# loop-Z/omniisaacgymenvs_loop

Hardware: AMD Instinct MI355X
Metric: env-steps/sec USV_CaptureXY at 1/2/4/8 MI355X; wall-clock to reward=30 (higher is better)
Workload: dtype fp32; 1 GPU; USV_Virtual_CaptureXY num_envs=131072/GPU PPO-MLP fp32 (BASELINE configs[4] per GPU: 2^20 envs over 8 GPUs); num_envs_per_gpu=131072, horizon_length=16, minibatch_size=8192, mini_epochs=8, parallelism=dp1, exchange=none (one rank), seed=0, full=False

## Files before the change

omniisaacgymenvs_loop_amd/csrc/ppo.hip:

```cpp
#include <cstdlib>
#include <cstring>
#include <type_traits>

#include "usv_device.h"

USV_PROBE_DEFINE(ppo)
USV_PROBE_DEFINE(pol)
USV_PROBE_DEFINE(red)

namespace {

constexpr int NIN = PPO_NIN, NH = PPO_NH, NA = PPO_NA;
constexpr int RB = 32;
constexpr int TB = 256;
constexpr int XS = 35;
constexpr int HS = 129;
constexpr int NPART = PPO_NPARAM + 8;
constexpr int NPART_PAD = (NPART + 3) & ~3;
constexpr int P_LOSS = PPO_NPARAM;
constexpr float kLog2Pi = 1.8378770664093453f;

typedef float f32x16 __attribute__((ext_vector_type(16)));
typedef unsigned int u32x4_t __attribute__((ext_vector_type(4)));

// ... 797 lines not shown
#pragma unroll
      for (int u = 0; u < 8; ++u) xv[u] = obs[(size_t)min(r0 + u * nl, bnd - 1) * NIN + col];
#pragma unroll
      for (int u = 0; u < 8; ++u)
        if (r0 + u * nl < bnd) {
          const double x = xv[u];
          s += x; s2 += x * x;
        }
    }
    acc[0][col][lane_r] = s;
    acc[1][col][lane_r] = s2;
  }
  __syncthreads();
  if (tid < NIN) {
    double t = 0, t2 = 0;
    for (int l = 0; l < nl; ++l) { t += acc[0][tid][l]; t2 += acc[1][tid][l]; }
    double *o = part + ((size_t)mb * OM_CH + ch) * 2 * NIN;
    o[tid] = t;
    o[NIN + tid] = t2;
  }
}

constexpr int RS_TB = 256, RS_U = 8;
__global__ __launch_bounds__(RS_TB) void k_obs_rms_seq(ppo_cfg_t c, const double *__restrict__ part, int nmb,
                                                       double *obs_rms, double *seq) {
  const double rows = (double)c.minibatch;
  for (int q = threadIdx.x; q < nmb * NIN; q += RS_TB) {
    const int mb = q / NIN, k = q % NIN;
    double sa = 0, sb = 0;
#pragma unroll
    for (int ch = 0; ch < OM_CH; ++ch) {
      const double *o = part + ((size_t)mb * OM_CH + ch) * 2 * NIN;
      sa += o[k];
      sb += o[NIN + k];
    }
    const double bmean = sa / rows;
    seq[(size_t)mb * 2 * NIN + k] = bmean;
    seq[(size_t)mb * 2 * NIN + NIN + k] = (sb - rows * bmean * bmean) / (rows - 1.0);
  }
  __syncthreads();
  const int k = threadIdx.x;
  if (k < NIN) {
    double mean = obs_rms[k], var = obs_rms[NIN + k], count = obs_rms[2 * NIN];
    for (int mb0 = 0; mb0 < nmb; mb0 += RS_U) {
      double bm[RS_U], bv[RS_U];
#pragma unroll
      for (int u = 0; u < RS_U; ++u) {
        const int mb = min(mb0 + u, nmb - 1);
        bm[u] = seq[(size_t)mb * 2 * NIN + k];
        bv[u] = seq[(size_t)mb * 2 * NIN + NIN + k];
      }
#pragma unroll
      for (int u = 0; u < RS_U; ++u) {
        if (mb0 + u >= nmb) break;
        const double tot = count + rows;
        const double delta = bm[u] - mean;
        const double M2 = var * count + bv[u] * rows + delta * delta * count * rows / tot;
        mean = mean + delta * rows / tot;
        var = M2 / tot;
        count = tot;
        seq[(size_t)(mb0 + u) * 2 * NIN + k] = mean;
        seq[(size_t)(mb0 + u) * 2 * NIN + NIN + k] = var;
      }
    }
    obs_rms[k] = mean;
    obs_rms[NIN + k] = var;
    if (k == 0) obs_rms[2 * NIN] = count;
  }
}

constexpr int GTB = 512;

#ifndef USV_RD_P
#define USV_RD_P 128
#endif
typedef float f32x4v __attribute__((ext_vector_type(4)));
constexpr int RD_TB = 512, RD_P = USV_RD_P;
constexpr int RD_L = RD_P / 4;
constexpr int RD_G = (RD_TB / RD_L);
constexpr int RD_KB = 16;
constexpr int RED_BLOCKS = (PPO_NPARAM + 5 + RD_P - 1) / RD_P;
static_assert(RD_P % 4 == 0 && 64 % RD_L == 0 && RD_P <= RD_TB, "reduce geometry");
static_assert(RED_BLOCKS <= 256, "chunk squares: one per thread of waves 0-3");

struct AdamBanks {
  const float *P0, *m0, *v0;
  float *P1, *m1, *v1;
};
struct AdamK {
  float step_size, bc2s;
};
__device__ __forceinline__ AdamK adam_consts(const ppo_cfg_t &c, float lr, float step) {
  const double bc1 = 1.0 - pow((double)c.adam_b1, (double)step);
  const double bc2 = 1.0 - pow((double)c.adam_b2, (double)step);
  return {(float)((double)lr / bc1), (float)sqrt(bc2)};
}
__device__ __forceinline__ void adam_one(const ppo_cfg_t &c, const AdamK &k, float g, float p_old, float m_old,
                                         float v_old, float &pn, float &mn, float &vn) {
  if (c.weight_decay != 0.f) g = g + c.weight_decay * p_old;
  mn = m_old + (1.0f - c.adam_b1) * (g - m_old);
  vn = v_old * c.adam_b2 + (1.0f - c.adam_b2) * g * g;
  const float denom = sqrtf(vn) / k.bc2s + c.adam_eps;
  pn = p_old - k.step_size * (mn / denom);
}
__device__ __forceinline__ float clip_coef(const ppo_cfg_t &c, float total_norm) {
  float coef = 1.0f;
  if (c.truncate_grads) {
    coef = c.grad_norm / (total_norm + 1e-6f);
    coef = fminf(coef, 1.0f);
  }
  return coef;
}
__device__ __forceinline__ AdamK adam_consts_tagged(const ppo_cfg_t &c, float lr, float step, float t_ss,
                                                    float t_bc, float t_step, float t_lr) {
  if (t_step == step && t_lr == lr) return {t_ss, t_bc};
  return adam_consts(c, lr, step);
}
struct OptNext {
  float nl, kl_keep, step;
  AdamK nk;
};
template <class OptIn>
__device__ __forceinline__ OptNext opt_next(const ppo_cfg_t &c, const OptIn &opt_in, float kl) {
  const float lr = opt_in[0];
  float nl = lr, kl_keep = opt_in[2];
  if (c.lr_adaptive) {
    if (kl > 2.0f * c.kl_threshold) nl = fmaxf(lr / 1.5f, c.lr_min);
    if (kl < 0.5f * c.kl_threshold) nl = fminf(lr * 1.5f, c.lr_max);
    kl_keep = kl;
  }
  const float step = opt_in[1] + 1.0f;
  return {nl, kl_keep, step, adam_consts(c, nl, step + 1.0f)};
}
__device__ __forceinline__ void opt_store(const ppo_cfg_t &c, const OptNext &x, float *opt_out, float total_norm,
                                          float kl, float *kl_out) {
  if (c.lr_adaptive && kl_out) *kl_out = kl;
  opt_out[0] = x.nl;
  opt_out[1] = x.step;
  opt_out[2] = x.kl_keep;
  opt_out[3] = total_norm;
  opt_out[4] = x.nk.step_size;
  opt_out[5] = x.nk.bc2s;
  opt_out[6] = x.step + 1.0f;
  opt_out[7] = x.nl;
}

struct ChainIn {
  const float *P_prev, *m_prev, *v_prev;
  float *P_cur, *m_cur, *v_cur;
  const float *grad;
  const float *opt_prev;
  float *opt_cur;
  float *kl_out;
  uint32_t *dp_clock;
  int fold_skip;
  float gscale;
};

constexpr int XG = XS;
constexpr int GX = ((RB * XG + GTB - 1) / GTB) * GTB;
struct GradSmem {
  float w2[NH * HS];
  float w1[NH * XG];
  float x[GX];
  float h1[RB * HS];
  float h2[RB * HS];
  float xch[4][16][64];
  float out[RB * 4];
  float g[RB * 4];
  float hg[4][4][NH];
  float b1[NH];
  float tail[TAIL + 1];
  float nrm[4];
  int fold[2];
};

constexpr int S_W2 = 0, S_W1 = NH * NH, S_SIG = S_W1 + NH * 32, S_B1 = S_SIG + 2, S_TAIL = S_B1 + NH,
              S_W1C = S_TAIL + TAIL, S_END = S_W1C + NH;
static_assert(S_END == PPO_NPARAM && S_W1 % 4 == 0 && NIN == 33, "partial slot layout");
__device__ __forceinline__ int tail_slot(int param) { return S_TAIL + param - PPO_OFF_B2; }
__device__ __forceinline__ int acc_slot(int base, int tile, int a, int lane) { return base + ((tile * 4 + a) * 64 + lane) * 4; }
__device__ __forceinline__ int param_of_slot(int s) {
  if (s < S_W1) {
    const int tile = s >> 10, a = (s >> 8) & 3, lane = (s >> 2) & 63, q = 4 * a + (s & 3);
    const int n = 32 * (tile >> 2) + crow(q, lane >> 5), k = 32 * (tile & 3) + (lane & 31);
    return PPO_OFF_W2 + n * NH + k;
  }
  if (s < S_SIG) {
    const int t = s - S_W1, tile = t >> 10, a = (t >> 8) & 3, lane = (t >> 2) & 63, q = 4 * a + (t & 3);
    const int n = 32 * tile + crow(q, lane >> 5), k = lane & 31;
    return PPO_OFF_W1 + n * NIN + k;
  }
  if (s < S_B1) return PPO_OFF_SIGMA + (s - S_SIG);
  if (s < S_TAIL) return PPO_OFF_B1 + (s - S_B1);
  if (s < S_W1C) return PPO_OFF_B2 + (s - S_TAIL);
  if (s < S_END) return PPO_OFF_W1 + (s - S_W1C) * NIN + (NIN - 1);
  return -1;
}

struct RowIn {
  float act0, act1, nlp, val, ret, adv, mu0, mu1, sg0, sg1;
};

#ifndef USV_PART_AUX
#define USV_PART_AUX 2
#endif
template <int kAux, bool kCM>
struct PartOutT {
  __amdgpu_buffer_rsrc_t r;
  uint32_t cs;
  __device__ __forceinline__ uint32_t off(int idx) const {
    if constexpr (kCM) return (uint32_t)(idx / RD_P) * cs + (uint32_t)(idx % RD_P) * 4u;
    else return (uint32_t)idx * 4u;
  }
  __device__ __forceinline__ void operator()(int idx, float v) const {
    __builtin_amdgcn_raw_buffer_store_b32(__builtin_bit_cast(uint32_t, v), r, off(idx), 0, kAux);
  }
  __device__ __forceinline__ void x4(int idx, float a, float b, float c, float d) const {
    const u32x4_t v = {__builtin_bit_cast(uint32_t, a), __builtin_bit_cast(uint32_t, b), __builtin_bit_cast(uint32_t, c),
                       __builtin_bit_cast(uint32_t, d)};
    __builtin_amdgcn_raw_buffer_store_b128(v, r, off(idx), 0, kAux);
  }
};
constexpr int AUX_SC1 = 16;

constexpr int FOLD_G = 8;
static_assert(RD_G >= FOLD_G, "k_reduce_partials(fold = 1) reads one group row per row group");
constexpr int FOLD_MAX_M = 32;
constexpr int FOLD_CTL_STRIDE = 64;
constexpr uint64_t FOLD_WAIT_TICKS = 10000;
__host__ __device__ constexpr size_t part_body_floats(int nblk) {
  return (size_t)nblk * RED_BLOCKS * RD_P > (size_t)(nblk + FOLD_G) * NPART_PAD ? (size_t)nblk * RED_BLOCKS * RD_P
                                                                                 : (size_t)(nblk + FOLD_G) * NPART_PAD;
}
__device__ __forceinline__ uint32_t *fold_ctl(float *partials, int nblk) {
  return reinterpret_cast<uint32_t *>(partials + part_body_floats(nblk));
}
__device__ __forceinline__ const uint32_t *fold_ctl(const float *partials, int nblk) {
  return reinterpret_cast<const uint32_t *>(partials + part_body_floats(nblk));
}
__device__ __forceinline__ f32x4v ld4_sc1(__amdgpu_buffer_rsrc_t r, uint32_t byte_off) {
  return __builtin_bit_cast(f32x4v, __builtin_amdgcn_raw_buffer_load_b128(r, byte_off, 0, AUX_SC1));
}

__device__ __forceinline__ void redo_step(const ppo_cfg_t &c, const ChainIn &ch, const float (&op)[8], float coef,
                                          float scale, GradSmem &s, float &ls0, float &ls1) {
  const AdamK ak = adam_consts_tagged(c, op[0], op[1] + 1.0f, op[4], op[5], op[6], op[7]);
  for (int q = threadIdx.x; q < PPO_NPARAM; q += GTB) {
    float pn, mn, vn;
    adam_one(c, ak, ch.grad[q] * scale * coef, ch.P_prev[q], ch.m_prev[q], ch.v_prev[q], pn, mn, vn);
    if ((q / GTB) % gridDim.x == blockIdx.x) {
      ch.P_cur[q] = pn; ch.m_cur[q] = mn; ch.v_cur[q] = vn;
    }
    if (q >= PPO_OFF_B2) {
      s.tail[q - PPO_OFF_B2] = pn;
    } else if (q >= PPO_OFF_W2) {
      const int e = q - PPO_OFF_W2;
      s.w2[(e / NH) * HS + e % NH] = pn;
    } else if (q >= PPO_OFF_B1) {
      s.b1[q - PPO_OFF_B1] = pn;
    } else if (q >= PPO_OFF_W1) {
      const int e = q - PPO_OFF_W1;
      s.w1[(e / NIN) * XG + e % NIN] = pn;
    }
  }
  float pn, mn, vn;
  adam_one(c, ak, ch.grad[PPO_OFF_SIGMA] * scale * coef, ch.P_prev[PPO_OFF_SIGMA], ch.m_prev[PPO_OFF_SIGMA],
           ch.v_prev[PPO_OFF_SIGMA], pn, mn, vn);
  ls0 = pn;
  adam_one(c, ak, ch.grad[PPO_OFF_SIGMA + 1] * scale * coef, ch.P_prev[PPO_OFF_SIGMA + 1],
           ch.m_prev[PPO_OFF_SIGMA + 1], ch.v_prev[PPO_OFF_SIGMA + 1], pn, mn, vn);
  ls1 = pn;
}

constexpr int APN_TB = 256;
__device__ __forceinline__ float apply_norm_part(const float *__restrict__ grad_in, float grad_scale, int tid) {
  constexpr int N4 = PPO_NPARAM / 4, U = (N4 + APN_TB - 1) / APN_TB;
  const float4 *g4 = reinterpret_cast<const float4 *>(grad_in);
  float4 gv[U];
#pragma unroll
  for (int u = 0; u < U; ++u) gv[u] = g4[min(tid + u * APN_TB, N4 - 1)];
  float ss = 0.f;
#pragma unroll
  for (int u = 0; u < U; ++u) {
    if (tid + u * APN_TB >= N4) continue;
    const float x = gv[u].x * grad_scale, y = gv[u].y * grad_scale;
    const float z = gv[u].z * grad_scale, w = gv[u].w * grad_scale;
    ss = fmaf(x, x, ss); ss = fmaf(y, y, ss); ss = fmaf(z, z, ss); ss = fmaf(w, w, ss);
  }
  for (int r = 4 * N4 + tid; r < PPO_NPARAM; r += APN_TB) {
    const float g = grad_in[r] * grad_scale;
    ss = fmaf(g, g, ss);
  }
  return ss;
}

template <bool kBf, bool kChain, bool kFold, bool kColl = false>
__device__ __forceinline__ void mb_grad8w(const ppo_cfg_t &c, const ChainIn &ch, const float *__restrict__ P,
                                          const double *__restrict__ obs_rms, int row0,
                                          const float *__restrict__ e_obs, const float *__restrict__ e_act,
                                          const float *__restrict__ e_nlp, const float *__restrict__ e_val,
                                          const float *__restrict__ e_ret, const float *__restrict__ e_adv,
                                          float *e_mu, float *e_sigma, float *partials, GradSmem &s) {
  const int tid = threadIdx.x, lane = tid & 63, w = tid >> 6;
  const int i = lane & 31, h = lane >> 5;
  const int kh = w >> 2, cb = w & 3, n0 = 32 * cb;
  const int rb0 = row0 + blockIdx.x * RB;
  const float invB = 1.0f / (float)c.minibatch;
  USV_PHASE(ppo, 0);
  if (ch.dp_clock && blockIdx.x == 0 && tid == 0) *ch.dp_clock += 1u;
  constexpr int NW1G = (NH * XG + GTB - 1) / GTB, NTLG = (TAIL + GTB - 1) / GTB, NW2F = NH * NH / GTB;
  static_assert(NH * NH % GTB == 0, "staging trip counts");
  float w2f[NW2F];
  float w1r[NW1G], tlr[NTLG];
  float ov = 0.f;
  if constexpr (kChain) ov = lane < 8 ? ch.opt_prev[lane] : ch.grad[PPO_NPARAM];
  {
#pragma unroll
    for (int u = 0; u < NW1G; ++u) {
      const int q = min(tid + u * GTB, NH * XG - 1), j = q / XG, k = q % XG;
      w1r[u] = P[PPO_OFF_W1 + j * NIN + min(k, NIN - 1)];
    }
#pragma unroll
    for (int u = 0; u < NTLG; ++u) tlr[u] = P[PPO_OFF_B2 + min(tid + u * GTB, TAIL - 1)];
  }
  const float b1r = P[PPO_OFF_B1 + (tid & (NH - 1))];
  const float lsv = P[PPO_OFF_SIGMA + (lane & 1)];
  float lsig0 = 0.f, lsig1 = 0.f;
  float csq = 0.f;
  if constexpr (kChain) csq = ch.grad[PPO_NPARAM + 8 + min(tid, RED_BLOCKS - 1)];
  RowIn ri;
  {
    const size_t row = (size_t)rb0 + (lane & (RB - 1));
    ri.act0 = e_act[row * 2]; ri.act1 = e_act[row * 2 + 1];
    ri.nlp = e_nlp[row]; ri.adv = e_adv[row];
    ri.val = e_val[row]; ri.ret = e_ret[row];
    ri.mu0 = e_mu[row * 2]; ri.mu1 = e_mu[row * 2 + 1];
    ri.sg0 = e_sigma[row * 2]; ri.sg1 = e_sigma[row * 2 + 1];
  }
  constexpr int NU = (RB * XG + GTB - 1) / GTB;
  float xo[NU];
  double mu[NU], var[NU];
#pragma unroll
  for (int u = 0; u < NU; ++u) {
    const int q = min(tid + u * GTB, RB * XG - 1), r = q / XG, kc = min(q % XG, NIN - 1);
    xo[u] = e_obs[(size_t)(rb0 + r) * NIN + kc];
    mu[u] = obs_rms[kc];
    var[u] = obs_rms[NIN + kc];
  }
#pragma unroll
  for (int u = 0; u < NW2F; ++u) w2f[u] = P[PPO_OFF_W2 + tid + u * GTB];
  __builtin_amdgcn_sched_barrier(0);
#pragma unroll
  for (int u = 0; u < NW1G; ++u)
    if ((tid + u * GTB) % XG >= NIN) w1r[u] = 0.f;
  if (kChain && tid >= RED_BLOCKS) csq = 0.f;
  {
    const bool norm = c.normalize_input != 0;
#pragma unroll
    for (int u = 0; u < NU; ++u) {
      const int q = tid + u * GTB;
      const int k = q % XG;
      const float xn = rms_norm(xo[u], mu[u], var[u], c.rms_eps);
      const float xv = (k < NIN && q < RB * XG) ? (norm ? xn : xo[u]) : 0.f;
      s.x[q] = xv;
    }
  }
#pragma unroll
  for (int u = 0; u < NW1G; ++u)
    if (tid + u * GTB < NH * XG) s.w1[tid + u * GTB] = w1r[u];
#pragma unroll
  for (int u = 0; u < NTLG; ++u)
    if (tid + u * GTB < TAIL) s.tail[tid + u * GTB] = tlr[u];
  if (tid < NH) s.b1[tid] = b1r;
  if (kChain && !kColl && w < 4) {
    const float t = wave_sum(csq);
    if (lane == 0) s.nrm[w] = t;
  }
  __syncthreads();
  if constexpr (kColl) {
    if (w < 4) {
      const float t = wave_sum(apply_norm_part(ch.grad, ch.gscale, tid));
      if (lane == 0) s.nrm[w] = t;
    }
    __syncthreads();
  }
  bool slow = false;
  if constexpr (kChain) {
    const auto lane_of = [&](int q) {
      return __builtin_bit_cast(float, __builtin_amdgcn_readlane(__builtin_bit_cast(int, ov), q));
    };
    const float total_norm = sqrtf(((s.nrm[0] + s.nrm[1]) + s.nrm[2]) + s.nrm[3]);
    const float coef = clip_coef(c, total_norm);
    const float gscale = kColl ? ch.gscale : 1.0f;
    if (blockIdx.x == 0 && tid == 256) {
      float op[8];
#pragma unroll
      for (int q = 0; q < 8; ++q) op[q] = lane_of(q);
      const float kl_prev = kColl ? lane_of(8) * gscale : lane_of(8);
      opt_store(c, opt_next(c, op, kl_prev), ch.opt_cur, total_norm, kl_prev, ch.kl_out);
    }
    if (kColl || coef < 1.0f) {
      slow = true;
      float op[8];
#pragma unroll
      for (int q = 0; q < 8; ++q) op[q] = lane_of(q);
      redo_step(c, ch, op, coef, gscale, s, lsig0, lsig1);
      __syncthreads();
    }
  }
  USV_PHASE(ppo, 1);
  if (kh == 0) {
    f32x16 acc = {};
#pragma unroll
    for (int st = 0; st < 17; ++st) {
      const int k = 2 * st + h;
      acc = mfma32(s.x[i * XG + k], s.w1[(n0 + i) * XG + k], acc);
    }
    const float bj = s.b1[n0 + i];
#pragma unroll
    for (int r = 0; r < 16; ++r) s.h1[crow(r, h) * HS + n0 + i] = fast_tanh(acc[r] + bj);
  }
  USV_PHASE(ppo, 9);
  if (!slow) {
#pragma unroll
    for (int u = 0; u < NW2F; ++u) {
      const int e = tid + u * GTB;
      s.w2[(e >> 7) * HS + (e & (NH - 1))] = w2f[u];
    }
  }
  __syncthreads();
  USV_PHASE(ppo, 10);
  const int ra = (i + 16 * kh) & (RB - 1);
  {
    f32x16 acc = {};
    if constexpr (kBf) {
#pragma unroll
      for (int st = 0; st < NH / 32; ++st) {
        const int k0 = 64 * kh + 16 * st + 8 * h;
        acc = mfma_bf16(ld8(&s.h1[ra * HS + k0]), ld8(&s.w2[(n0 + i) * HS + k0]), acc);
      }
    } else {
#pragma unroll 16
      for (int st = 0; st < NH / 4; ++st) {
        const int k = 64 * kh + 2 * st + h;
        acc = mfma32(s.h1[ra * HS + k], s.w2[(n0 + i) * HS + k], acc);
      }
    }
    USV_PHASE(ppo, 11);
#pragma unroll
    for (int q = 0; q < 8; ++q) s.xch[cb][8 * kh + q][lane] = acc[8 + q];
    __syncthreads();
    const float bj = s.tail[T_B2 + n0 + i];
#pragma unroll
    for (int q = 0; q < 8; ++q)
      s.h2[(crow(q, h) + 16 * kh) * HS + n0 + i] = fast_tanh((acc[q] + s.xch[cb][8 - 8 * kh + q][lane]) + bj);
  }
  __syncthreads();
  USV_PHASE(ppo, 12);
  constexpr bool kCM = !kFold;
  const PartOutT<kFold ? AUX_SC1 : USV_PART_AUX, kCM> part_st{
      kCM ? __builtin_amdgcn_make_buffer_rsrc(partials + (size_t)blockIdx.x * RD_P, 0,
                                              (int)(((size_t)RED_BLOCKS * gridDim.x - blockIdx.x) * RD_P * 4), 0x00020000)
          : __builtin_amdgcn_make_buffer_rsrc(partials + (size_t)blockIdx.x * NPART_PAD, 0, NPART * 4, 0x00020000),
      (uint32_t)gridDim.x * RD_P * 4u};
  {
    const int r = tid / 16, part = tid % 16;
    float a0 = 0.f, a1 = 0.f, av = 0.f;
#pragma unroll
    for (int kk = 0; kk < 8; ++kk) {
      const int k = part + 16 * kk;
      const float hv = s.h2[r * HS + k];
      a0 = fmaf(s.tail[T_WMU + k], hv, a0);
      a1 = fmaf(s.tail[T_WMU + NH + k], hv, a1);
      av = fmaf(s.tail[T_WV + k], hv, av);
    }
#pragma unroll
    for (int m = 1; m < 16; m <<= 1) {
      a0 += __shfl_xor(a0, m, 64);
      a1 += __shfl_xor(a1, m, 64);
      av += __shfl_xor(av, m, 64);
    }
    if (part == 0) {
      s.out[r * 4 + 0] = a0 + s.tail[T_BMU];
      s.out[r * 4 + 1] = a1 + s.tail[T_BMU + 1];
      s.out[r * 4 + 2] = av + s.tail[T_BV];
    }
  }
  __syncthreads();
  USV_PHASE(ppo, 2);
  if (tid < 192) {
    const int r = lane;
    const bool rowok = r < RB;
    const int rr = rowok ? r : 0;
    const size_t row = (size_t)rb0 + rr;
    const float mu0 = s.out[rr * 4], mu1 = s.out[rr * 4 + 1], v = s.out[rr * 4 + 2];
    if (!slow) {
      lsig0 = __builtin_bit_cast(float, __builtin_amdgcn_readlane(__builtin_bit_cast(int, lsv), 0));
      lsig1 = __builtin_bit_cast(float, __builtin_amdgcn_readlane(__builtin_bit_cast(int, lsv), 1));
    }
    const float ls0 = mu0 * 0.f + lsig0, ls1 = mu1 * 0.f + lsig1;
    const float sg0 = expf(ls0), sg1 = expf(ls1);
    const float bh0 = fmaxf(mu0 - 1.1f, 0.f), bl0 = fminf(mu0 + 1.1f, 0.f);
    const float bh1 = fmaxf(mu1 - 1.1f, 0.f), bl1 = fminf(mu1 + 1.1f, 0.f);
    if (w == 0) {
      float la = 0.f, gs0 = 0.f, gs1 = 0.f;
      if (rowok) {
// ... 363 lines not shown
  const int p4 = blockIdx.x * RD_L + col;
  const bool ok = p4 < NPART_PAD / 4;
  const float4 *P4 = reinterpret_cast<const float4 *>(partials);
  const int myslot = blockIdx.x * RD_P + tid;
  const bool mine = kSpec && tid < RD_P && myslot < S_END;
  const int pq = mine ? param_of_slot(myslot) : 0;
  float p_old = 0.f, m_old = 0.f, v_old = 0.f;
  if (mine) {
    p_old = a.P0[pq]; m_old = a.m0[pq]; v_old = a.v0[pq];
  }
  uint32_t key = 0u;
  if (kDP) key = *dp.clock;
  float4 acc = make_float4(0.f, 0.f, 0.f, 0.f);
  float oin[8] = {};
  if (kSpec) {
#pragma unroll
    for (int q = 0; q < 8; ++q) oin[q] = opt_in[q];
  }
  const int p4c = min(p4, NPART_PAD / 4 - 1);
  if (fold) {
    if (grp < FOLD_G) {
      const int M = nblk / FOLD_G;
      const uint32_t *ctl = fold_ctl(partials, nblk) + grp * FOLD_CTL_STRIDE;
      const uint32_t gen = ctl[0] / (uint32_t)M;
      bool folded = true;
      for (int mm = 0; mm < M; ++mm) folded &= ctl[32 + mm] == gen;
      if (folded) {
        acc = P4[(size_t)(nblk + grp) * (NPART_PAD / 4) + p4c];
      } else {
        const int h0 = (M + 1) / 2;
        float4 a0 = make_float4(0.f, 0.f, 0.f, 0.f), a1 = a0;
        for (int mm = 0; mm < M; ++mm) {
          const float4 x = P4[(size_t)(grp + FOLD_G * mm) * (NPART_PAD / 4) + p4c];
          float4 &t = mm < h0 ? a0 : a1;
          t.x += x.x; t.y += x.y; t.z += x.z; t.w += x.w;
        }
        acc = make_float4(a0.x + a1.x, a0.y + a1.y, a0.z + a1.z, a0.w + a1.w);
      }
    }
  } else
  for (int b0 = grp; b0 < nblk; b0 += RD_G * RD_KB) {
    float4 x[RD_KB];
#pragma unroll
    for (int k = 0; k < RD_KB; ++k) {
      const int row = min(b0 + RD_G * k, nblk - 1);
      const float4 *src = P4 + ((size_t)blockIdx.x * nblk + row) * RD_L + col;
      const f32x4v v = __builtin_nontemporal_load(reinterpret_cast<const f32x4v *>(src));
      x[k] = make_float4(v[0], v[1], v[2], v[3]);
    }
#pragma unroll
    for (int k = 0; k < RD_KB; ++k) {
      if (ok && b0 + RD_G * k < nblk) {
        acc.x += x[k].x; acc.y += x[k].y; acc.z += x[k].z; acc.w += x[k].w;
      }
    }
  }
  USV_PHASE(red, 1);
  AdamK ak = {0.f, 1.f};
  if (kSpec)
    ak = adam_consts_tagged(c, oin[0], oin[1] + 1.0f, oin[4], oin[5], oin[6], oin[7]);
  red[grp][col] = acc;
  __syncthreads();
  float s = 0.f;
  const int slot = blockIdx.x * RD_P + tid;
  if (tid < RD_P) {
#pragma unroll
    for (int g = 0; g < RD_G; ++g) s += reinterpret_cast<const float *>(red[g])[tid];
  }
  USV_PHASE(red, 2);
  float sl = s;
  if constexpr (kDP) {
    const float pv = slot < S_END ? s : (slot == PPO_NPARAM + 4 ? s * inv_b : 0.f);
    s = dp_exchange(dp, key, blockIdx.x, slot, pv, dp.timeout_ms) / (float)dp.world;
  }
  float sq = 0.f;
  if (tid < RD_P) {
    if (slot < S_END) {
      grad[param_of_slot(slot)] = s;
      sq = s * s;
      if (mine) {
        float pn, mn, vn;
        adam_one(c, ak, s, p_old, m_old, v_old, pn, mn, vn);
        a.P1[pq] = pn; a.m1[pq] = mn; a.v1[pq] = vn;
      }
    } else if (slot < PPO_NPARAM + 5) {
      const int q = slot - PPO_NPARAM;
      if (q == 4) grad[PPO_NPARAM] = kDP ? s : s * inv_b;
      if (losses) losses[q] = sl * inv_b;
    }
  }
  USV_PHASE(red, 3);
  if (w < (RD_P + 63) / 64) {
    sq = wave_sum(sq);
    if (lane == 0) sqw[w] = sq;
  }
  __syncthreads();
  if (tid == 0) {
    float t = 0.f;
#pragma unroll
    for (int q = 0; q < (RD_P + 63) / 64; ++q) t += sqw[q];
    grad[PPO_NPARAM + 8 + blockIdx.x] = t;
  }
  USV_PHASE(red, 4);
}

constexpr int AP_TB = 256;
template <bool kNormFromPartials, bool kFinish>
__global__ __launch_bounds__(AP_TB) void k_apply(ppo_cfg_t c, AdamBanks a, const float *__restrict__ grad_in,
                                                 const float *__restrict__ opt_in, float *__restrict__ opt_out,
                                                 float grad_scale, float *kl_out) {
  __shared__ float red[AP_TB / 64];
  const int tid = threadIdx.x;
  const int q = blockIdx.x * AP_TB + tid;
  const int qc = min(q, PPO_NPARAM - 1);
  const float g_raw = grad_in[qc], p_old = a.P0[qc], m_old = a.m0[qc], v_old = a.v0[qc];
  const float s0 = grad_in[PPO_NPARAM + 8 + min(tid, RED_BLOCKS - 1)];
  const float lr = opt_in[0];
  const float step = opt_in[1] + 1.0f;
  const float kl = grad_in[PPO_NPARAM] * grad_scale;
  __builtin_amdgcn_sched_barrier(0);
  const AdamK ak = adam_consts_tagged(c, lr, step, opt_in[4], opt_in[5], opt_in[6], opt_in[7]);
  OptNext nx = {};
  if (blockIdx.x == 0 && tid == 0) nx = opt_next(c, opt_in, kl);
  __asm__ volatile("" : : "v"(ak.step_size), "v"(ak.bc2s), "v"(nx.nl), "v"(nx.nk.step_size), "v"(nx.nk.bc2s));
  float ss = 0.f;
  if (kNormFromPartials) {
    ss = tid < RED_BLOCKS ? s0 : 0.f;
  } else {
    constexpr int N4 = PPO_NPARAM / 4, U = (N4 + AP_TB - 1) / AP_TB;
    const float4 *g4 = reinterpret_cast<const float4 *>(grad_in);
    float4 gv[U];
#pragma unroll
    for (int u = 0; u < U; ++u) gv[u] = g4[min(tid + u * AP_TB, N4 - 1)];
#pragma unroll
    for (int u = 0; u < U; ++u) {
      if (tid + u * AP_TB >= N4) continue;
      const float x = gv[u].x * grad_scale, y = gv[u].y * grad_scale;
      const float z = gv[u].z * grad_scale, w = gv[u].w * grad_scale;
      ss = fmaf(x, x, ss); ss = fmaf(y, y, ss); ss = fmaf(z, z, ss); ss = fmaf(w, w, ss);
    }
    for (int r = 4 * N4 + tid; r < PPO_NPARAM; r += AP_TB) {
      const float g = grad_in[r] * grad_scale;
      ss = fmaf(g, g, ss);
    }
  }
  ss = wave_sum(ss);
  if ((tid & 63) == 0) red[tid >> 6] = ss;
  __syncthreads();
  const float total_norm = sqrtf(((red[0] + red[1]) + red[2]) + red[3]);
  const float coef = clip_coef(c, total_norm);
  if (q < PPO_NPARAM && (!kFinish || coef < 1.0f)) {
    float pn, mn, vn;
    adam_one(c, ak, g_raw * grad_scale * coef, p_old, m_old, v_old, pn, mn, vn);
    a.P1[q] = pn;
    a.m1[q] = mn;
    a.v1[q] = vn;
  }
  if (blockIdx.x == 0 && tid == 0) opt_store(c, nx, opt_out, total_norm, kl, kl_out);
}

}

extern "C" {

int ppo_policy_step(const ppo_cfg_t *cfg, const float *params, const double *obs_rms, const double *val_rms,
                    const float *obs, int t, float *exp_obs, float *exp_act, float *exp_nlp, float *exp_val,
// ... 48 lines not shown
                const float *last_obs, const int64_t *last_dones, const uint8_t *exp_done, float *exp_val,
                const float *exp_rew, float *exp_ret, float *exp_adv, double *work, void *stream) {
  if (!cfg || !params || !work || cfg->n_envs <= 0) return 1;
  hipStream_t s = (hipStream_t)stream;
  float *last_val = reinterpret_cast<float *>(work + 8 + 8 * 4096);
  if (ppo_value(cfg, params, obs_rms, val_rms, last_obs, last_val, stream)) return 2;
  const int nblk = (cfg->n_envs + TB - 1) / TB;
  if (nblk > 4096) return 3;
  const char *gv = getenv("USV_GAE_VEC");
  const bool vec16 = !(gv && atoi(gv) == 0) && cfg->horizon == 16 &&
                     ((reinterpret_cast<uintptr_t>(exp_val) | reinterpret_cast<uintptr_t>(exp_rew) |
                       reinterpret_cast<uintptr_t>(exp_ret) | reinterpret_cast<uintptr_t>(exp_adv) |
                       reinterpret_cast<uintptr_t>(exp_done)) & 15u) == 0;
  hipLaunchKernelGGL(vec16 ? k_gae<16> : k_gae<0>, dim3(nblk), dim3(TB), 0, s, *cfg, last_val, last_dones, exp_done,
                     exp_val, exp_rew, exp_ret, exp_adv, work);
  USV_CHECK_LAUNCH();
  hipLaunchKernelGGL(k_prepare_finalize, dim3(1), dim3(FIN_TB), 0, s, *cfg, val_rms, work, nblk);
  USV_CHECK_LAUNCH();
  const size_t B = (size_t)cfg->n_envs * cfg->horizon;
  hipLaunchKernelGGL(k_prepare_apply, dim3((unsigned)((B + 255) / 256)), dim3(256), 0, s, *cfg, work, exp_val,
                     exp_ret, exp_adv);
  USV_CHECK_LAUNCH();
  return 0;
}

static int fold_env() {
  const char *e = getenv("USV_PPO_FOLD");
  return e ? atoi(e) : 0;
}
static bool fold_on(int nblk) {
  return fold_env() != 0 && nblk % FOLD_G == 0 && nblk / FOLD_G >= 1 && nblk / FOLD_G <= FOLD_MAX_M;
}

int ppo_minibatch_grad(const ppo_cfg_t *cfg, const float *params, double *obs_rms, const double *val_rms,
                       int update_obs_rms, int mb_index, const float *exp_obs, const float *exp_act,
                       const float *exp_nlp, const float *exp_val, const float *exp_ret, const float *exp_adv,
                       float *exp_mu, float *exp_sigma, float *grad, float *losses, float *partials, double *work,
                       void *stream) {
  (void)val_rms;
  if (!cfg || !params || !obs_rms || !grad || !partials || !work) return 1;
  if (cfg->minibatch % RB != 0 || ppo_partials_floats(cfg->minibatch) <= 0) return 2;
  if (reinterpret_cast<uintptr_t>(params) & 15u) return 4;
  hipStream_t s = (hipStream_t)stream;
  const int row0 = mb_index * cfg->minibatch;
  if (update_obs_rms && cfg->normalize_input) {
    const int nb = 64;
    hipLaunchKernelGGL(k_obs_stats, dim3(nb), dim3(TB), 0, s, *cfg, exp_obs, row0, cfg->minibatch, work + 8, obs_rms,
                       reinterpret_cast<unsigned *>(work + 7));
    USV_CHECK_LAUNCH();
  }
  if (reinterpret_cast<uintptr_t>(partials) & 15u) return 3;
  const int nblk = cfg->minibatch / RB;
  const bool fold = fold_on(nblk);
  ChainIn ch{};
  ch.fold_skip = fold_env() == 2;
  hipLaunchKernelGGL((cfg->bf16_gemm ? (fold ? k_mb_grad<true, false, true> : k_mb_grad<true, false, false>)
                                     : (fold ? k_mb_grad<false, false, true> : k_mb_grad<false, false, false>)),
                     dim3(nblk), dim3(GTB), 0, s, *cfg, ch, params, obs_rms, row0, exp_obs, exp_act, exp_nlp,
                     exp_val, exp_ret, exp_adv, exp_mu, exp_sigma, partials);
  USV_CHECK_LAUNCH();
  hipLaunchKernelGGL((k_reduce_partials<false, false>), dim3(RED_BLOCKS), dim3(RD_TB), 0, s, partials, nblk, grad,
                     losses, 1.0f / (float)cfg->minibatch, *cfg, AdamBanks{}, nullptr, ppo_dp_t{}, (int)fold);
  USV_CHECK_LAUNCH();
  return 0;
}

static bool banks_ok(const ppo_adam_banks_t *b) {
  if (!b || !b->opt) return false;
  for (int i = 0; i < 2; ++i) {
    if (!b->params[i] || !b->m[i] || !b->v[i]) return false;
    if (reinterpret_cast<uintptr_t>(b->params[i]) & 15u) return false;
  }
  return true;
}

static int fused_launch(const ppo_cfg_t *cfg, const ppo_adam_banks_t *banks, const ppo_dp_t *dp, int seq,
                        double *obs_rms, int update_obs_rms, int mb_index, const float *exp_obs, const float *exp_act,
                        const float *exp_nlp, const float *exp_val, const float *exp_ret, const float *exp_adv,
                        float *exp_mu, float *exp_sigma, float *grad, float *losses, float *partials, double *work,
                        float *kl_prev_out, void *stream) {
  if (!cfg || !obs_rms || !grad || !partials || !work || seq < 0) return 1;
  if (!banks_ok(banks)) return 4;
  if (cfg->minibatch % RB != 0 || ppo_partials_floats(cfg->minibatch) <= 0) return 2;
  if (reinterpret_cast<uintptr_t>(partials) & 15u) return 3;
  if (dp) {
    if (dp->world < 1 || dp->world > PPO_DP_MAX || dp->rank < 0 || dp->rank >= dp->world || !dp->clock || !dp->err)
      return 5;
    for (int r = 0; r < dp->world; ++r)
      if (!dp->peer[r]) return 5;
  }
  hipStream_t s = (hipStream_t)stream;
  const int cur = seq & 1, prv = cur ^ 1, nblk = cfg->minibatch / RB, row0 = mb_index * cfg->minibatch;
  if (update_obs_rms && cfg->normalize_input) {
    hipLaunchKernelGGL(k_obs_stats, dim3(64), dim3(TB), 0, s, *cfg, exp_obs, row0, cfg->minibatch, work + 8, obs_rms,
                       reinterpret_cast<unsigned *>(work + 7));
    USV_CHECK_LAUNCH();
  }
  const float *P = banks->params[cur];
  const dim3 gg(nblk), gb(GTB);
  uint32_t *clk = dp ? dp->clock : nullptr;
  const bool fold = fold_on(nblk);
  if (seq == 0) {
    ChainIn ch{};
    ch.dp_clock = clk;
    ch.fold_skip = fold_env() == 2;
    hipLaunchKernelGGL((cfg->bf16_gemm ? (fold ? k_mb_grad<true, false, true> : k_mb_grad<true, false, false>)
                                       : (fold ? k_mb_grad<false, false, true> : k_mb_grad<false, false, false>)),
                       gg, gb, 0, s, *cfg, ch, P, obs_rms, row0, exp_obs, exp_act, exp_nlp, exp_val, exp_ret, exp_adv,
                       exp_mu, exp_sigma, partials);
  } else {
    const ChainIn ch{banks->params[prv], banks->m[prv], banks->v[prv], banks->params[cur], banks->m[cur],
                     banks->v[cur], grad, banks->opt + 8 * prv, banks->opt + 8 * cur, kl_prev_out, clk,
                     fold_env() == 2};
    hipLaunchKernelGGL((cfg->bf16_gemm ? (fold ? k_mb_grad<true, true, true> : k_mb_grad<true, true, false>)
                                       : (fold ? k_mb_grad<false, true, true> : k_mb_grad<false, true, false>)),
                       gg, gb, 0, s, *cfg, ch, P, obs_rms, row0, exp_obs, exp_act, exp_nlp, exp_val, exp_ret, exp_adv,
                       exp_mu, exp_sigma, partials);
  }
  USV_CHECK_LAUNCH();
  const AdamBanks a{banks->params[cur], banks->m[cur], banks->v[cur], banks->params[prv], banks->m[prv],
                    banks->v[prv]};
  if (dp)
    hipLaunchKernelGGL((k_reduce_partials<true, true>), dim3(RED_BLOCKS), dim3(RD_TB), 0, s, partials, nblk, grad,
                       losses, 1.0f / (float)cfg->minibatch, *cfg, a, banks->opt + 8 * cur, *dp, (int)fold);
  else
    hipLaunchKernelGGL((k_reduce_partials<true, false>), dim3(RED_BLOCKS), dim3(RD_TB), 0, s, partials, nblk, grad,
                       losses, 1.0f / (float)cfg->minibatch, *cfg, a, banks->opt + 8 * cur, ppo_dp_t{}, (int)fold);
  USV_CHECK_LAUNCH();
  return 0;
}

int ppo_minibatch_fused(const ppo_cfg_t *cfg, const ppo_adam_banks_t *banks, int seq, double *obs_rms,
                        int update_obs_rms, int mb_index, const float *exp_obs, const float *exp_act,
                        const float *exp_nlp, const float *exp_val, const float *exp_ret, const float *exp_adv,
                        float *exp_mu, float *exp_sigma, float *grad, float *losses, float *partials, double *work,
                        float *kl_prev_out, void *stream) {
  return fused_launch(cfg, banks, nullptr, seq, obs_rms, update_obs_rms, mb_index, exp_obs, exp_act, exp_nlp, exp_val,
                      exp_ret, exp_adv, exp_mu, exp_sigma, grad, losses, partials, work, kl_prev_out, stream);
}

int ppo_minibatch_fused_dp(const ppo_cfg_t *cfg, const ppo_adam_banks_t *banks, const ppo_dp_t *dp, int seq,
                           double *obs_rms, int update_obs_rms, int mb_index, const float *exp_obs,
                           const float *exp_act, const float *exp_nlp, const float *exp_val, const float *exp_ret,
                           const float *exp_adv, float *exp_mu, float *exp_sigma, float *grad, float *losses,
                           float *partials, double *work, float *kl_prev_out, void *stream) {
  if (!dp) return 5;
  return fused_launch(cfg, banks, dp, seq, obs_rms, update_obs_rms, mb_index, exp_obs, exp_act, exp_nlp, exp_val,
                      exp_ret, exp_adv, exp_mu, exp_sigma, grad, losses, partials, work, kl_prev_out, stream);
}

int ppo_minibatch_coll(const ppo_cfg_t *cfg, const ppo_adam_banks_t *banks, int seq, float grad_scale,
                       double *obs_rms, int update_obs_rms, int mb_index, const float *exp_obs, const float *exp_act,
                       const float *exp_nlp, const float *exp_val, const float *exp_ret, const float *exp_adv,
                       float *exp_mu, float *exp_sigma, float *grad, float *losses, float *partials, double *work,
                       float *kl_prev_out, void *stream) {
  if (!cfg || !obs_rms || !grad || !partials || !work || seq < 0 || !(grad_scale > 0.f)) return 1;
  if (!banks_ok(banks)) return 4;
  if (cfg->minibatch % RB != 0 || ppo_partials_floats(cfg->minibatch) <= 0) return 2;
  if ((reinterpret_cast<uintptr_t>(partials) | reinterpret_cast<uintptr_t>(grad)) & 15u) return 3;
  hipStream_t s = (hipStream_t)stream;
  const int cur = seq & 1, prv = cur ^ 1, nblk = cfg->minibatch / RB, row0 = mb_index * cfg->minibatch;
  if (update_obs_rms && cfg->normalize_input) {
    hipLaunchKernelGGL(k_obs_stats, dim3(64), dim3(TB), 0, s, *cfg, exp_obs, row0, cfg->minibatch, work + 8, obs_rms,
                       reinterpret_cast<unsigned *>(work + 7));
    USV_CHECK_LAUNCH();
  }
  const float *P = banks->params[cur];
// ... 43 lines not shown
  hipLaunchKernelGGL(k_dp_selftest, dim3(RED_BLOCKS), dim3(RD_TB), 0, (hipStream_t)stream, *dp, (uint32_t)key0,
                     rounds, timeout_ms);
  USV_CHECK_LAUNCH();
  return 0;
}

int ppo_dp_alloc(void **dptr, void *ipc_handle) {
  if (!dptr || !ipc_handle) return 1;
  static_assert(sizeof(hipIpcMemHandle_t) == 64, "ipc handle size");
  const char *mode = getenv("USV_DP_MALLOC");
  const bool plain = mode && strcmp(mode, "plain") == 0;
  if (plain || hipExtMallocWithFlags(dptr, (size_t)DP_BYTES, hipDeviceMallocUncached) != hipSuccess) {
    (void)hipGetLastError();
    if (hipMalloc(dptr, (size_t)DP_BYTES) != hipSuccess) return 2;
  }
  if (hipMemset(*dptr, 0, (size_t)DP_BYTES) != hipSuccess || hipDeviceSynchronize() != hipSuccess) return 3;
  hipIpcMemHandle_t h;
  if (hipIpcGetMemHandle(&h, *dptr) != hipSuccess) return 4;
  memcpy(ipc_handle, &h, sizeof(h));
  return 0;
}

int ppo_dp_open(const void *ipc_handle, void **dptr) {
  if (!dptr || !ipc_handle) return 1;
  hipIpcMemHandle_t h;
  memcpy(&h, ipc_handle, sizeof(h));
  return hipIpcOpenMemHandle(dptr, h, hipIpcMemLazyEnablePeerAccess) == hipSuccess ? 0 : 2;
}

int ppo_dp_close(void *dptr) { return hipIpcCloseMemHandle(dptr) == hipSuccess ? 0 : 1; }
int ppo_dp_free(void *dptr) { return hipFree(dptr) == hipSuccess ? 0 : 1; }

int ppo_minibatch_finish(const ppo_cfg_t *cfg, const ppo_adam_banks_t *banks, int count, const float *grad,
                         float *kl_out, void *stream) {
  if (!cfg || !grad || count <= 0) return 1;
  if (!banks_ok(banks)) return 4;
  const int last = (count - 1) & 1, nxt = last ^ 1;
  const AdamBanks a{banks->params[last], banks->m[last], banks->v[last], banks->params[nxt], banks->m[nxt],
                    banks->v[nxt]};
  hipLaunchKernelGGL((k_apply<true, true>), dim3((PPO_NPARAM + AP_TB - 1) / AP_TB), dim3(AP_TB), 0,
                     (hipStream_t)stream, *cfg, a, grad, banks->opt + 8 * last, banks->opt + 8 * nxt, 1.0f, kl_out);
  USV_CHECK_LAUNCH();
  return 0;
}

int ppo_rms_seq_doubles(const ppo_cfg_t *cfg, int rows) {
  if (!cfg || cfg->minibatch <= 0 || rows < cfg->minibatch) return -1;
  const int nmb = rows / cfg->minibatch;
  return nmb * 2 * NIN + nmb * OM_CH * 2 * NIN;
}

int ppo_obs_rms_epoch(const ppo_cfg_t *cfg, const float *exp_obs, int rows, double *obs_rms, double *rms_seq,
                      void *stream) {
  if (!cfg || !exp_obs || !obs_rms || !rms_seq || cfg->minibatch <= 1 || rows < cfg->minibatch) return 1;
  const int nmb = rows / cfg->minibatch;
  hipStream_t s = (hipStream_t)stream;
  double *part = rms_seq + (size_t)nmb * 2 * NIN;
  hipLaunchKernelGGL(k_obs_moments, dim3(nmb, OM_CH), dim3(TB), 0, s, *cfg, exp_obs, part);
  USV_CHECK_LAUNCH();
  hipLaunchKernelGGL(k_obs_rms_seq, dim3(1), dim3(RS_TB), 0, s, *cfg, part, nmb, obs_rms, rms_seq);
  USV_CHECK_LAUNCH();
  return 0;
}

int ppo_minibatch_apply(const ppo_cfg_t *cfg, float *params, float *grad, float *adam_m, float *adam_v, float *opt,
                        int opt_slot, float grad_scale, float *kl_out, int norm_from_partials, void *stream) {
  if (!cfg || !params || !grad || !adam_m || !adam_v || !opt) return 1;
  if (reinterpret_cast<uintptr_t>(grad) & 15u) return 2;
  if (opt_slot != 0 && opt_slot != 1) return 3;
  const AdamBanks a{params, adam_m, adam_v, params, adam_m, adam_v};
  hipLaunchKernelGGL((norm_from_partials ? k_apply<true, false> : k_apply<false, false>),
                     dim3((PPO_NPARAM + AP_TB - 1) / AP_TB), dim3(AP_TB), 0, (hipStream_t)stream, *cfg, a, grad,
                     opt + 8 * opt_slot, opt + 8 * (1 - opt_slot), grad_scale, kl_out);
  USV_CHECK_LAUNCH();
  return 0;
}

int ppo_partials_floats(int minibatch) {
  static_assert(RED_BLOCKS * RD_P >= NPART_PAD, "chunk-major rows cover a partial row");
  if (minibatch < RB || minibatch % RB != 0) return -1;
  const long long f = (long long)part_body_floats(minibatch / RB) + FOLD_G * FOLD_CTL_STRIDE;
  return f > 0x7fffffffLL ? -1 : (int)f;
}
int ppo_grad_floats(void) { return PPO_NPARAM + 8 + RED_BLOCKS; }
int ppo_meter_floats(int n_envs, int horizon) {
  return horizon * 4 + horizon * ((n_envs + kStoreTB - 1) / kStoreTB) * 4;
}

}
```

Baseline: 35.36 million env-steps/s.

## Stage W2 into LDS via direct global-to-LDS DMA from padded image

The reduce/Adam kernel now also writes updated W2 weights into a padded, LDS-layout image appended to the grad buffer. The chained gradient kernel then copies that image straight into shared memory with global_load_lds_dwordx4, instead of loading W2 into registers and scattering it to LDS later. This is meant to cut register pressure and the VGPR-to-LDS store pass, and to overlap the W2 load with the layer-1 compute. In exchange it adds extra global writes in the reduce kernel, a larger grad buffer, inline asm that touches m0, and explicit vmcnt waits.

```diff
diff --git a/omniisaacgymenvs_loop_amd/csrc/ppo.hip b/omniisaacgymenvs_loop_amd/csrc/ppo.hip
--- a/omniisaacgymenvs_loop_amd/csrc/ppo.hip
+++ b/omniisaacgymenvs_loop_amd/csrc/ppo.hip
@@ -903,6 +903,12 @@
 constexpr int RED_BLOCKS = (PPO_NPARAM + 5 + RD_P - 1) / RD_P;
 static_assert(RD_P % 4 == 0 && 64 % RD_L == 0 && RD_P <= RD_TB, "reduce geometry");
 static_assert(RED_BLOCKS <= 256, "chunk squares: one per thread of waves 0-3");
+constexpr int W2IMG_FLOATS = (NH * HS + 3) & ~3;
+constexpr int W2IMG_OFF = (PPO_NPARAM + 8 + RED_BLOCKS + 3) & ~3;
+constexpr int W2IMG_PIECES = W2IMG_FLOATS / 256;
+constexpr int W2IMG_LAST_LANES = W2IMG_FLOATS % 256 / 4;
+static_assert(W2IMG_FLOATS == NH * HS && W2IMG_PIECES % 8 == 0 && W2IMG_LAST_LANES > 0 && W2IMG_LAST_LANES < 64,
+              "W2 image: the copy covers s.w2 exactly, 8 waves x whole pieces + one partial piece");
 
 struct AdamBanks {
   const float *P0, *m0, *v0;
@@ -981,7 +987,7 @@
 constexpr int XG = XS;
 constexpr int GX = ((RB * XG + GTB - 1) / GTB) * GTB;
 struct GradSmem {
-  float w2[NH * HS];
+  alignas(16) float w2[NH * HS];
   float w1[NH * XG];
   float x[GX];
   float h1[RB * HS];
@@ -1062,6 +1068,15 @@
 }
 __device__ __forceinline__ f32x4v ld4_sc1(__amdgpu_buffer_rsrc_t r, uint32_t byte_off) {
   return __builtin_bit_cast(f32x4v, __builtin_amdgcn_raw_buffer_load_b128(r, byte_off, 0, AUX_SC1));
+}
+
+__device__ __forceinline__ void lds_dma16(const float *src, uint32_t lds_dst) {
+  uint32_t keep;
+  __asm__ volatile("s_mov_b32 %0, m0\n\ts_mov_b32 m0, %2\n\ts_nop 0\n\tglobal_load_lds_dwordx4 %1, off\n\t"
+                   "s_mov_b32 m0, %0"
+                   : "=&s"(keep)
+                   : "v"(src), "s"(lds_dst)
+                   : "memory");
 }
 
 __device__ __forceinline__ void redo_step(const ppo_cfg_t &c, const ChainIn &ch, const float (&op)[8], float coef,
@@ -1132,7 +1147,8 @@
   if (ch.dp_clock && blockIdx.x == 0 && tid == 0) *ch.dp_clock += 1u;
   constexpr int NW1G = (NH * XG + GTB - 1) / GTB, NTLG = (TAIL + GTB - 1) / GTB, NW2F = NH * NH / GTB;
   static_assert(NH * NH % GTB == 0, "staging trip counts");
-  float w2f[NW2F];
+  constexpr bool kImg = kChain && !kColl && !kFold;
+  float w2f[kImg ? 1 : NW2F];
   float w1r[NW1G], tlr[NTLG];
   float ov = 0.f;
   if constexpr (kChain) ov = lane < 8 ? ch.opt_prev[lane] : ch.grad[PPO_NPARAM];
@@ -1146,19 +1162,21 @@
     for (int u = 0; u < NTLG; ++u) tlr[u] = P[PPO_OFF_B2 + min(tid + u * GTB, TAIL - 1)];
   }
   const float b1r = P[PPO_OFF_B1 + (tid & (NH - 1))];
-  const float lsv = P[PPO_OFF_SIGMA + (lane & 1)];
+  float lsv;
+  if constexpr (!kImg) lsv = P[PPO_OFF_SIGMA + (lane & 1)];
   float lsig0 = 0.f, lsig1 = 0.f;
   float csq = 0.f;
   if constexpr (kChain) csq = ch.grad[PPO_NPARAM + 8 + min(tid, RED_BLOCKS - 1)];
   RowIn ri;
-  {
+  const auto load_rows = [&] {
     const size_t row = (size_t)rb0 + (lane & (RB - 1));
     ri.act0 = e_act[row * 2]; ri.act1 = e_act[row * 2 + 1];
     ri.nlp = e_nlp[row]; ri.adv = e_adv[row];
     ri.val = e_val[row]; ri.ret = e_ret[row];
     ri.mu0 = e_mu[row * 2]; ri.mu1 = e_mu[row * 2 + 1];
     ri.sg0 = e_sigma[row * 2]; ri.sg1 = e_sigma[row * 2 + 1];
-  }
+  };
+  if constexpr (!kImg) load_rows();
   constexpr int NU = (RB * XG + GTB - 1) / GTB;
   float xo[NU];
   double mu[NU], var[NU];
@@ -1169,8 +1187,23 @@
     mu[u] = obs_rms[kc];
     var[u] = obs_rms[NIN + kc];
   }
-#pragma unroll
-  for (int u = 0; u < NW2F; ++u) w2f[u] = P[PPO_OFF_W2 + tid + u * GTB];
+  if constexpr (kImg) {
+    lsv = P[PPO_OFF_SIGMA + (lane & 1)];
+    load_rows();
+    const int wu = __builtin_amdgcn_readfirstlane(w);
+    const uint32_t w2lds = (uint32_t)(uintptr_t)(__attribute__((address_space(3))) float *)s.w2;
+    const float *img = ch.grad + W2IMG_OFF + lane * 4;
+    if (wu == GTB / 64 - 1 && lane < W2IMG_LAST_LANES)
+      lds_dma16(img + W2IMG_PIECES * 256, w2lds + W2IMG_PIECES * 1024);
+#pragma unroll
+    for (int u = 0; u < W2IMG_PIECES / (GTB / 64); ++u) {
+      const int pc = wu + (GTB / 64) * u;
+      lds_dma16(img + pc * 256, w2lds + pc * 1024);
+    }
+  } else {
+#pragma unroll
+    for (int u = 0; u < NW2F; ++u) w2f[u] = P[PPO_OFF_W2 + tid + u * GTB];
+  }
   __builtin_amdgcn_sched_barrier(0);
 #pragma unroll
   for (int u = 0; u < NW1G; ++u)
@@ -1223,6 +1256,10 @@
     }
     if (kColl || coef < 1.0f) {
       slow = true;
+      if constexpr (kImg) {
+        __asm__ volatile("s_waitcnt vmcnt(0)" ::: "memory");
+        __syncthreads();
+      }
       float op[8];
 #pragma unroll
       for (int q = 0; q < 8; ++q) op[q] = lane_of(q);
@@ -1243,7 +1280,9 @@
     for (int r = 0; r < 16; ++r) s.h1[crow(r, h) * HS + n0 + i] = fast_tanh(acc[r] + bj);
   }
   USV_PHASE(ppo, 9);
-  if (!slow) {
+  if constexpr (kImg) {
+    __asm__ volatile("s_waitcnt vmcnt(0)" ::: "memory");
+  } else if (!slow) {
 #pragma unroll
     for (int u = 0; u < NW2F; ++u) {
       const int e = tid + u * GTB;
@@ -1773,6 +1812,10 @@
         float pn, mn, vn;
         adam_one(c, ak, s, p_old, m_old, v_old, pn, mn, vn);
         a.P1[pq] = pn; a.m1[pq] = mn; a.v1[pq] = vn;
+        if (pq >= PPO_OFF_W2 && pq < PPO_OFF_B2) {
+          const int e = pq - PPO_OFF_W2;
+          grad[W2IMG_OFF + (e / NH) * HS + e % NH] = pn;
+        }
       }
     } else if (slot < PPO_NPARAM + 5) {
       const int q = slot - PPO_NPARAM;
@@ -1987,7 +2030,7 @@
   if (!cfg || !obs_rms || !grad || !partials || !work || seq < 0) return 1;
   if (!banks_ok(banks)) return 4;
   if (cfg->minibatch % RB != 0 || ppo_partials_floats(cfg->minibatch) <= 0) return 2;
-  if (reinterpret_cast<uintptr_t>(partials) & 15u) return 3;
+  if ((reinterpret_cast<uintptr_t>(partials) | reinterpret_cast<uintptr_t>(grad)) & 15u) return 3;
   if (dp) {
     if (dp->world < 1 || dp->world > PPO_DP_MAX || dp->rank < 0 || dp->rank >= dp->world || !dp->clock || !dp->err)
       return 5;
@@ -2197,7 +2240,7 @@
   const long long f = (long long)part_body_floats(minibatch / RB) + FOLD_G * FOLD_CTL_STRIDE;
   return f > 0x7fffffffLL ? -1 : (int)f;
 }
-int ppo_grad_floats(void) { return PPO_NPARAM + 8 + RED_BLOCKS; }
+int ppo_grad_floats(void) { return W2IMG_OFF + W2IMG_FLOATS; }
 int ppo_meter_floats(int n_envs, int horizon) {
   return horizon * 4 + horizon * ((n_envs + kStoreTB - 1) / kStoreTB) * 4;
 }
```

Result: no change. 36.07 million env-steps/s (median of 6 runs) (+2.0%).
